# playHing/Scaled-MMD-GAN

Measured on AMD Instinct MI355X. Metric: images/sec/step (64x64 SMMD, batch 64) + MMD-kernel GB/s at 1/2/4/8 GPU, higher is better.
Workload: dtype fp32; 1 GPU; imagenet_smmd 64x64 SNResNet G/D, rbf kernel, scaling, SN, batch 64/GPU, 5D+1G schedule; model=snresnet, global_batch=64, parallelism=dp1, dp_mode=global, dp_forced=False, memory_format=nchw, miopen_winograd=True, miopen_find=False, step_graphs=False, conv_mean_pool=folded 4x4 stride-2 conv, miopen_db=/tmp/code/home/pair/home_parent/tmp/smmd_miopen_db_0gvd9db2

## Files before the change

### include/smmd_hip.h

```cpp
#ifndef SMMD_HIP_H
#define SMMD_HIP_H

#include <stddef.h>
#include <stdint.h>

#ifdef __cplusplus
extern "C" {
#endif

typedef enum {
    SMMD_OK = 0,
    SMMD_EINVAL = 1,
    SMMD_EHIP = 2,
    SMMD_EWORKSPACE = 3,
    SMMD_EUNSUPPORTED = 4
} smmd_status;

typedef void *smmd_stream_t;

typedef enum {
    SMMD_KIND_RBF = 0,
    SMMD_KIND_RQ = 1,
    SMMD_KIND_DISTANCE = 2,
    SMMD_KIND_DOT = 3
// ... 245 lines not shown
smmd_status smmd_cond_bn_relu_fwd(const float *x, const int32_t *labels, int N, int C, int HW,
                                  int num_classes, const float *scale, const float *offset,
                                  float eps, float *y, float *save, void *ws, size_t ws_bytes,
                                  smmd_stream_t stream);

smmd_status smmd_cond_bn_relu_bwd(const float *x, const float *gy, const int32_t *labels, int N,
                                  int C, int HW, int num_classes, const float *scale,
                                  const float *offset, const float *save, float *gx, float *gscale,
                                  float *goffset, void *ws, size_t ws_bytes, smmd_stream_t stream);

smmd_status smmd_conv3x3_thin(const float *x, const float *w, const float *bias, float *y,
                              int n, int ci, int co, int h, int w_img, int mode,
                              smmd_stream_t stream);

size_t smmd_conv3x3_thin_wgrad_workspace_bytes(int n, int ci, int co, int h, int w_img);

smmd_status smmd_conv3x3_thin_wgrad(const float *gy, const float *x, float *gw, int n, int ci,
                                    int co, int h, int w_img, void *ws, size_t ws_bytes,
                                    smmd_stream_t stream);

smmd_status smmd_conv3x3_thin_wgrad_acc(const float *gy, const float *x, float *gw, int n,
                                        int ci, int co, int h, int w_img, void *ws,
                                        size_t ws_bytes, smmd_stream_t stream);

int smmd_wino3x3_supported(int n, int ci, int ko, int h, int w_img);

size_t smmd_wino3x3_filter_bytes(int ko, int ci);

smmd_status smmd_wino3x3_filter(const float *w, int ko, int ci, int mode, float *u,
                                size_t u_bytes, smmd_stream_t stream);

size_t smmd_wino3x3_workspace_bytes(int n, int ci, int ko, int h, int w_img);

smmd_status smmd_wino3x3_conv(const float *x, const float *u, const float *bias, float *y, int n,
                              int ci, int ko, int h, int w_img, void *ws, size_t ws_bytes,
                              smmd_stream_t stream);

smmd_status smmd_wino3x3_conv_relu(const float *x, const float *u, const float *bias, float *y,
                                   int n, int ci, int ko, int h, int w_img, void *ws,
                                   size_t ws_bytes, smmd_stream_t stream);

smmd_status smmd_wino3x3_conv_mask(const float *x, const float *u, const float *bias,
                                   const float *mask, float *y, int n, int ci, int ko, int h,
                                   int w_img, void *ws, size_t ws_bytes, smmd_stream_t stream);

size_t smmd_wino3x3_conv2_workspace_bytes(int n, int ci, int ko, int h, int w_img);

smmd_status smmd_wino3x3_conv2(const float *x, const float *u, const float *x2, const float *u2,
                               const float *bias, float *y, int n, int ci, int ko, int h,
                               int w_img, void *ws, size_t ws_bytes, smmd_stream_t stream);

int smmd_wino4x4s2_supported(int n, int ci, int ko, int h, int w_img);

int smmd_wino4x4s2t_supported(int n, int k, int c, int hg, int wg);

size_t smmd_wino4x4s2_filter_bytes(int ko, int ci);

smmd_status smmd_wino4x4s2_filter(const float *w, int ko, int ci, float *u, size_t u_bytes,
                                  smmd_stream_t stream);

smmd_status smmd_wino4x4s2t_filter(const float *w, int k, int c, float *u, size_t u_bytes,
                                   smmd_stream_t stream);

size_t smmd_wino4x4s2_workspace_bytes(int n, int ci, int ko, int h, int w_img);

size_t smmd_wino4x4s2t_workspace_bytes(int n, int k, int c, int hg, int wg);

smmd_status smmd_wino4x4s2_conv(const float *x, const float *u, const float *bias, float *y,
                                int n, int ci, int ko, int h, int w_img, void *ws,
                                size_t ws_bytes, smmd_stream_t stream);

smmd_status smmd_wino4x4s2_conv_acc(const float *x, const float *u, const float *bias, float *y,
                                    int n, int ci, int ko, int h, int w_img, void *ws,
                                    size_t ws_bytes, smmd_stream_t stream);

smmd_status smmd_wino4x4s2t_conv(const float *gy, const float *u, const float *bias, float *dx,
                                 int n, int k, int c, int hg, int wg, void *ws, size_t ws_bytes,
                                 smmd_stream_t stream);

smmd_status smmd_wino4x4s2t_conv_mask(const float *gy, const float *u, const float *bias,
                                      const float *mask, float *dx, int n, int k, int c, int hg,
                                      int wg, void *ws, size_t ws_bytes, smmd_stream_t stream);

size_t smmd_wino4x4s2_conv2_workspace_bytes(int n, int ci, int ko, int h, int w_img);

smmd_status smmd_wino4x4s2_conv2(const float *x, const float *u, const float *x2,
                                 const float *u2, const float *bias, float *y, int n, int ci,
                                 int ko, int h, int w_img, void *ws, size_t ws_bytes,
                                 smmd_stream_t stream);

smmd_status smmd_wino3x3_filter_sn(const float *w, const float *sigma, const float *s, int ko,
                                   int ci, int mode, float *u, size_t u_bytes,
                                   smmd_stream_t stream);

smmd_status smmd_wino4x4s2_filter_sn(const float *w, const float *sigma, const float *s, int fold,
                                     int ko, int ci, float *u, size_t u_bytes,
                                     smmd_stream_t stream);

smmd_status smmd_wino4x4s2t_filter_sn(const float *w, const float *sigma, const float *s,
                                      int fold, int k, int c, float *u, size_t u_bytes,
                                      smmd_stream_t stream);

int smmd_wino3x3_wgrad_supported(int n, int ci, int co, int h, int w_img);


size_t smmd_wino3x3_wgrad_workspace_bytes(int n, int ci, int co, int h, int w_img);

smmd_status smmd_wino3x3_wgrad(const float *x, const float *gy, float *gw, int n, int ci, int co,
                               int h, int w_img, void *ws, size_t ws_bytes,
                               smmd_stream_t stream);

smmd_status smmd_wino3x3_wgrad_acc(const float *x, const float *gy, float *gw, int n, int ci,
                                   int co, int h, int w_img, void *ws, size_t ws_bytes,
                                   smmd_stream_t stream);

int smmd_wino4x4s2_wgrad_supported(int n, int ci, int co, int h, int w_img);

size_t smmd_wino4x4s2_wgrad_workspace_bytes(int n, int ci, int co, int h, int w_img);

smmd_status smmd_wino4x4s2_wgrad(const float *x, const float *gy, float *gw, int n, int ci,
                                 int co, int h, int w_img, void *ws, size_t ws_bytes,
                                 smmd_stream_t stream);

smmd_status smmd_wino4x4s2_wgrad_acc(const float *x, const float *gy, float *gw, int n, int ci,
                                     int co, int h, int w_img, void *ws, size_t ws_bytes,
                                     smmd_stream_t stream);

int smmd_conv1x1_supported(int n, int r, int m, int p);

size_t smmd_conv1x1_workspace_bytes(int n, int r, int m, int p);

smmd_status smmd_conv1x1(const float *a, const float *x, const float *bias, float *y, int n,
                         int r, int m, int p, void *ws, size_t ws_bytes, smmd_stream_t stream);

smmd_status smmd_conv1x1_t(const float *a, const float *x, const float *bias, float *y, int n,
                           int r, int m, int p, void *ws, size_t ws_bytes, smmd_stream_t stream);

int smmd_conv1x1_wgrad_supported(int n, int c, int k, int p);

size_t smmd_conv1x1_wgrad_workspace_bytes(int n, int c, int k, int p);

smmd_status smmd_conv1x1_wgrad(const float *gy, const float *x, float *gw, int n, int c, int k,
                               int p, void *ws, size_t ws_bytes, smmd_stream_t stream);

smmd_status smmd_conv1x1_wgrad_acc(const float *gy, const float *x, float *gw, int n, int c,
                                   int k, int p, void *ws, size_t ws_bytes,
                                   smmd_stream_t stream);

smmd_status smmd_gp_interp(const float *real, const float *fake, const float *alpha, float *out,
                           int b, int64_t per, int form, smmd_stream_t stream);

size_t smmd_gp_slope_workspace_bytes(int b, int c, int hw);

smmd_status smmd_gp_slope_fwd(const float *g, int b, int c, int hw, int channels_last, float eps,
                              float *out, float *slopes, void *ws, size_t ws_bytes,
                              smmd_stream_t stream);

smmd_status smmd_gp_slope_bwd(const float *g, const float *slopes, int b, int c, int hw,
                              int channels_last, const float *go, float *dg,
                              smmd_stream_t stream);

smmd_status smmd_critic_head_fwd(const float *d_real, int n_real, const float *d_fake, int n_fake,
                                 int kind, float *out, float *g_real, float *g_fake,
                                 float *gg_fake, smmd_stream_t stream);

size_t smmd_code_moments_workspace_bytes(int n, int dim);
// ... 10 lines not shown
```

### scaled-mmd-gan_amd/csrc/smmd_wino_s2.hip

```cpp
#include "smmd_wino_common.hpp"
#include "smmd_ldsdma.hpp"

namespace smmd {

namespace {

constexpr int S2_T = 256;
constexpr int S2_TB = 64;
constexpr int S2_KB = 64;
constexpr int S2_CC = 2;
constexpr int S2_STAGE = 9 * 8 * 64;
constexpr size_t S2_LDS = 2 * 2 * S2_STAGE * sizeof(float) + S2_KB * sizeof(float);

struct for_wino4x4s2_conv {};
struct for_wino4x4s2t_conv {};

__device__ __forceinline__ void s2_taps(const float *__restrict__ w, int64_t q, int fold,
                                        const float *__restrict__ sig,
                                        const float *__restrict__ sc, float (&f)[16]) {
#pragma clang fp contract(off)
    if (!sig) {
        const float *s = w + q * 16;
#pragma unroll
        for (int i = 0; i < 16; ++i) f[i] = s[i];
        return;
    }
    const float sigma = sig[0], scale = sc ? sc[0] : 1.f;
    if (!fold) {
        const float *s = w + q * 16;
#pragma unroll
        for (int i = 0; i < 16; ++i) f[i] = (s[i] / sigma) * scale;
        return;
    }
    const float *s = w + q * 9;
    float k[9];
#pragma unroll
    for (int j = 0; j < 9; ++j) k[j] = (s[j] / sigma) * scale;
#pragma unroll
    for (int si = 0; si < 4; ++si)
#pragma unroll
        for (int ti = 0; ti < 4; ++ti) {
            float acc = 0.f;
#pragma unroll
            for (int a = 0; a < 2; ++a)
#pragma unroll
                for (int b = 0; b < 2; ++b) {
                    const int uu = si - a, vv = ti - b;
                    if (uu >= 0 && uu < 3 && vv >= 0 && vv < 3) acc += k[uu * 3 + vv];
                }
            f[si * 4 + ti] = acc * 0.25f;
        }
}

__global__ void s2_filter_kernel(const float *__restrict__ w, int KO, int CI,
                                 float *__restrict__ u, const float *__restrict__ sig,
                                 const float *__restrict__ sc, int fold) {
    const int64_t idx = (int64_t)blockIdx.x * blockDim.x + threadIdx.x;
    if (idx >= (int64_t)KO * CI) return;
    const int ko = (int)(idx % KO), ci = (int)(idx / KO);
    float f[16];
    s2_taps(w, (int64_t)ko * CI + ci, fold, sig, sc, f);
    const int kb = ko >> 6, kl = ko & 63, cc = ci >> 1, h = ci & 1;
    const int64_t base = ((int64_t)kb * (CI >> 1) + cc) * 9;
    float r[9][4];
#pragma unroll
    for (int pi = 0; pi < 2; ++pi)
#pragma unroll
        for (int pj = 0; pj < 2; ++pj) {
            const float g00 = f[(pi) * 4 + pj], g01 = f[(pi) * 4 + 2 + pj];
            const float g10 = f[(2 + pi) * 4 + pj], g11 = f[(2 + pi) * 4 + 2 + pj];
            const float t[3][2] = {{g00, g01}, {g00 + g10, g01 + g11}, {g10, g11}};
#pragma unroll
            for (int i = 0; i < 3; ++i) {
                r[i * 3 + 0][2 * pi + pj] = t[i][0];
                r[i * 3 + 1][2 * pi + pj] = t[i][0] + t[i][1];
                r[i * 3 + 2][2 * pi + pj] = t[i][1];
            }
        }
    float4 *u4 = reinterpret_cast<float4 *>(u);
#pragma unroll
    for (int p = 0; p < 9; ++p)
        u4[((base + p) * 2 + h) * 64 + kl] = make_float4(r[p][0], r[p][1], r[p][2], r[p][3]);
// ... 508 lines not shown
    }

    const int64_t et = tile0 + th * 32 + l32;
    if (et >= g.T) return;
    const int en = (int)(et / g.Timg);
    const int er = (int)(et - (int64_t)en * g.Timg);
    const int ety = er / g.TW, etx = er - ety * g.TW;
    const int Hx = 2 * g.Hg, Wx = 2 * g.Wg;
    const int cl0 = kh * 32 + 4 * hl;
    const uint32_t o0 = (uint32_t)(((((int64_t)en * g.C + cb * 64 + cl0) * Hx + 4 * ety + qi) * Wx +
                                     4 * etx + qj) * 4);
    const uint32_t o1 = o0 + (uint32_t)Wx * 8;
    const uint32_t hw4 = (uint32_t)Hx * (uint32_t)Wx * 4;
    const __amdgpu_buffer_rsrc_t ds = buf_rsrc_2g(dx);
    float mk[16][4];
    const bool masked = g.mask != nullptr;
    if (masked) {
        const __amdgpu_buffer_rsrc_t ms = buf_rsrc_2g(g.mask);
#pragma unroll
        for (int r = 0; r < 16; r += 2) {
#pragma unroll
            for (int h = 0; h < 2; ++h) {
                const uint32_t so = (uint32_t)((r & 3) + 8 * (r >> 2) + h) * hw4;
                mk[r + h][0] = __builtin_bit_cast(float, __builtin_amdgcn_raw_buffer_load_b32(ms, o0, so, 0));
                mk[r + h][1] = __builtin_bit_cast(float, __builtin_amdgcn_raw_buffer_load_b32(ms, o0 + 8, so, 0));
                mk[r + h][2] = __builtin_bit_cast(float, __builtin_amdgcn_raw_buffer_load_b32(ms, o1, so, 0));
                mk[r + h][3] = __builtin_bit_cast(float, __builtin_amdgcn_raw_buffer_load_b32(ms, o1 + 8, so, 0));
            }
        }
    }
#ifdef S2_NO_EPI
    for (int r = 0; r < 2; r += 2) {
#else
#pragma unroll
    for (int r = 0; r < 16; r += 2) {
#endif
        const int cr = (r & 3) + 8 * (r >> 2);
#pragma unroll
        for (int h = 0; h < 2; ++h) {
            float m[9];
#pragma unroll
            for (int p = 0; p < 9; ++p) m[p] = acc[p][r + h];
            float s0[3], s1[3];
#pragma unroll
            for (int j = 0; j < 3; ++j) {
                s0[j] = m[j] + m[3 + j];
                s1[j] = m[3 + j] + m[6 + j];
            }
            const float b = Bs[cl0 + cr + h];
            float v[4] = {s0[0] + s0[1] + b, s0[1] + s0[2] + b, s1[0] + s1[1] + b,
                          s1[1] + s1[2] + b};
            if (masked) {
#pragma unroll
                for (int i = 0; i < 4; ++i) v[i] = mk[r + h][i] <= 0.f ? 0.f : v[i];
            }
            const uint32_t so = (uint32_t)(cr + h) * hw4;
            __builtin_amdgcn_raw_buffer_store_b32(__builtin_bit_cast(unsigned, v[0]), ds, o0, so, 0);
            __builtin_amdgcn_raw_buffer_store_b32(__builtin_bit_cast(unsigned, v[1]), ds, o0 + 8, so, 0);
            __builtin_amdgcn_raw_buffer_store_b32(__builtin_bit_cast(unsigned, v[2]), ds, o1, so, 0);
            __builtin_amdgcn_raw_buffer_store_b32(__builtin_bit_cast(unsigned, v[3]), ds, o1 + 8, so, 0);
        }
    }
}

template <bool EDGE>
__global__ __launch_bounds__(S2_T, 2) void s2t_conv_kernel(
    const float *__restrict__ gy, const float *__restrict__ u, const float *__restrict__ bias,
    float *__restrict__ dx, S2TGeom g) {
    uint32_t W = s2_xcd_order(blockIdx.x, gridDim.x);
    const int q = (int)(W & 3);
    W >>= 2;
    const int cb = (int)(W % (uint32_t)g.CB);
    W /= (uint32_t)g.CB;
    const int sl = (int)(W % (uint32_t)g.S);
    const int64_t tb = W / (uint32_t)g.S;
    switch (q) {
    case 0: s2t_body<EDGE, 0, 0>(gy, u, bias, dx, g, tb, cb, sl); break;
    case 1: s2t_body<EDGE, 0, 1>(gy, u, bias, dx, g, tb, cb, sl); break;
    case 2: s2t_body<EDGE, 1, 0>(gy, u, bias, dx, g, tb, cb, sl); break;
    default: s2t_body<EDGE, 1, 1>(gy, u, bias, dx, g, tb, cb, sl); break;
    }
}

}

static int s2_target() { return 256; }

static int s2t_slices(int64_t blocks, int nch) {
    int S = 1;
    while (blocks * S < s2_target() && nch / (2 * S) >= 4) S *= 2;
    return S;
}

static int s2_slices(int64_t blocks, int nch, int HWo) {
    int S = 1;
    while (blocks * S < s2_target() && nch / (2 * S) >= 8 && HWo % 4 == 0) S *= 2;
    return S;
}

}

using namespace smmd;

extern "C" int smmd_wino4x4s2_supported(int n, int ci, int ko, int h, int w_img) {
    return n > 0 && ci > 0 && ko > 0 && ci % S2_CC == 0 && ko % S2_KB == 0 && h > 0 &&
           w_img > 0 && h % 4 == 0 && w_img % 4 == 0 && (int64_t)n * ci * h * w_img < (1ll << 29) &&
           (int64_t)n * ko * h * w_img < (1ll << 31);
}

extern "C" size_t smmd_wino4x4s2_filter_bytes(int ko, int ci) {
    if (ko <= 0 || ci <= 0) return 0;
    return (size_t)36 * ko * ci * sizeof(float);
}

extern "C" smmd_status smmd_wino4x4s2_filter(const float *w, int ko, int ci, float *u,
                                             size_t u_bytes, smmd_stream_t stream) {
    if (ko <= 0 || ci <= 0 || !w || !u) return SMMD_EINVAL;
    if (ko % S2_KB || ci % S2_CC) return SMMD_EUNSUPPORTED;
    if (reinterpret_cast<uintptr_t>(u) & 15) return SMMD_EINVAL;
    if (u_bytes < smmd_wino4x4s2_filter_bytes(ko, ci)) return SMMD_EWORKSPACE;
    hipStream_t st = reinterpret_cast<hipStream_t>(stream);
    const int64_t n = (int64_t)ko * ci;
    s2_filter_kernel<<<dim3((unsigned)((n + 255) / 256)), dim3(256), 0, st>>>(w, ko, ci, u,
                                                                             nullptr, nullptr, 0);
    return last_launch_status();
}

extern "C" smmd_status smmd_wino4x4s2_filter_sn(const float *w, const float *sigma,
                                                const float *s, int fold, int ko, int ci,
                                                float *u, size_t u_bytes, smmd_stream_t stream) {
    if (ko <= 0 || ci <= 0 || !w || !u || !sigma || (fold != 0 && fold != 1)) return SMMD_EINVAL;
    if (ko % S2_KB || ci % S2_CC) return SMMD_EUNSUPPORTED;
    if (reinterpret_cast<uintptr_t>(u) & 15) return SMMD_EINVAL;
    if (u_bytes < smmd_wino4x4s2_filter_bytes(ko, ci)) return SMMD_EWORKSPACE;
    hipStream_t st = reinterpret_cast<hipStream_t>(stream);
    const int64_t n = (int64_t)ko * ci;
    s2_filter_kernel<<<dim3((unsigned)((n + 255) / 256)), dim3(256), 0, st>>>(w, ko, ci, u,
                                                                             sigma, s, fold);
    return last_launch_status();
}

extern "C" size_t smmd_wino4x4s2_workspace_bytes(int n, int ci, int ko, int h, int w_img) {
    if (!smmd_wino4x4s2_supported(n, ci, ko, h, w_img)) return 0;
    const int64_t T = (int64_t)n * (h / 4) * (w_img / 4);
    const int S = s2_slices(((T + S2_TB - 1) / S2_TB) * (ko / S2_KB), ci / S2_CC,
                            (h / 2) * (w_img / 2));
    return S > 1 ? (size_t)S * n * ko * (h / 2) * (w_img / 2) * sizeof(float) : 0;
}

static smmd_status s2_conv(const float *x, const float *u, const float *x2, const float *u2,
                           const float *bias, float *y, int n, int ci, int ko, int h, int w_img,
                           void *ws, size_t ws_bytes, smmd_stream_t stream, int acc = 0) {
    if (n < 0 || ci <= 0 || ko <= 0 || h < 0 || w_img < 0) return SMMD_EINVAL;
    if (n == 0 || h == 0 || w_img == 0) return SMMD_OK;
    if (!x || !u || !y || (!x2 != !u2)) return SMMD_EINVAL;
    if (!smmd_wino4x4s2_supported(n, ci, ko, h, w_img)) return SMMD_EUNSUPPORTED;
    if ((reinterpret_cast<uintptr_t>(x) | reinterpret_cast<uintptr_t>(y) |
         reinterpret_cast<uintptr_t>(u) | reinterpret_cast<uintptr_t>(x2) |
         reinterpret_cast<uintptr_t>(u2)) & 15)
        return SMMD_EINVAL;
    const int pair = x2 ? 2 : 1;
    S2Geom g{};
    g.x2 = x2;
    g.u2 = u2;
    g.N = n; g.C = ci; g.K = ko; g.H = h; g.W = w_img;
    g.TW = w_img / 4;
    g.Timg = (h / 4) * g.TW;
    g.T = (int64_t)n * g.Timg;
    const int64_t tb = (g.T + S2_TB - 1) / S2_TB;
    if (tb > 0x7fffffff) return SMMD_EINVAL;
    const int HWo = (h / 2) * (w_img / 2);
    const int S = s2_slices(tb * (ko / S2_KB), pair * ci / S2_CC, HWo);
    const int64_t total = (int64_t)n * ko * HWo;
    float *out = y;
// ... 43 lines not shown
extern "C" size_t smmd_wino4x4s2_conv2_workspace_bytes(int n, int ci, int ko, int h, int w_img) {
    if (!smmd_wino4x4s2_supported(n, ci, ko, h, w_img)) return 0;
    const int64_t T = (int64_t)n * (h / 4) * (w_img / 4);
    const int S = s2_slices(((T + S2_TB - 1) / S2_TB) * (ko / S2_KB), 2 * ci / S2_CC,
                            (h / 2) * (w_img / 2));
    return S > 1 ? (size_t)S * n * ko * (h / 2) * (w_img / 2) * sizeof(float) : 0;
}

extern "C" smmd_status smmd_wino4x4s2_conv2(const float *x, const float *u, const float *x2,
                                            const float *u2, const float *bias, float *y, int n,
                                            int ci, int ko, int h, int w_img, void *ws,
                                            size_t ws_bytes, smmd_stream_t stream) {
    if (!x2 || !u2) return SMMD_EINVAL;
    return s2_conv(x, u, x2, u2, bias, y, n, ci, ko, h, w_img, ws, ws_bytes, stream);
}

extern "C" int smmd_wino4x4s2t_supported(int n, int k, int c, int hg, int wg) {
    return n > 0 && k > 0 && c > 0 && k % 8 == 0 && c % 64 == 0 && hg > 0 && wg > 0 &&
           hg % 2 == 0 && wg % 2 == 0 && (int64_t)n * k * hg * wg < (1ll << 29) &&
           (int64_t)n * c * 4 * hg * wg < (1ll << 29);
}

extern "C" smmd_status smmd_wino4x4s2t_filter(const float *w, int k, int c, float *u,
                                              size_t u_bytes, smmd_stream_t stream) {
    if (k <= 0 || c <= 0 || !w || !u) return SMMD_EINVAL;
    if (k % 8 || c % 64) return SMMD_EUNSUPPORTED;
    if (reinterpret_cast<uintptr_t>(u) & 15) return SMMD_EINVAL;
    if (u_bytes < smmd_wino4x4s2_filter_bytes(k, c)) return SMMD_EWORKSPACE;
    hipStream_t st = reinterpret_cast<hipStream_t>(stream);
    const int64_t n = (int64_t)(k / 4) * c;
    s2t_filter_kernel<<<dim3((unsigned)((n + 255) / 256)), dim3(256), 0, st>>>(w, k, c, u,
                                                                              nullptr, nullptr, 0);
    return last_launch_status();
}

extern "C" smmd_status smmd_wino4x4s2t_filter_sn(const float *w, const float *sigma,
                                                 const float *s, int fold, int k, int c,
                                                 float *u, size_t u_bytes, smmd_stream_t stream) {
    if (k <= 0 || c <= 0 || !w || !u || !sigma || (fold != 0 && fold != 1)) return SMMD_EINVAL;
    if (k % 8 || c % 64) return SMMD_EUNSUPPORTED;
    if (reinterpret_cast<uintptr_t>(u) & 15) return SMMD_EINVAL;
    if (u_bytes < smmd_wino4x4s2_filter_bytes(k, c)) return SMMD_EWORKSPACE;
    hipStream_t st = reinterpret_cast<hipStream_t>(stream);
    const int64_t n = (int64_t)(k / 4) * c;
    s2t_filter_kernel<<<dim3((unsigned)((n + 255) / 256)), dim3(256), 0, st>>>(w, k, c, u,
                                                                              sigma, s, fold);
    return last_launch_status();
}

extern "C" size_t smmd_wino4x4s2t_workspace_bytes(int n, int k, int c, int hg, int wg) {
    if (!smmd_wino4x4s2t_supported(n, k, c, hg, wg)) return 0;
    const int64_t T = (int64_t)n * (hg / 2) * (wg / 2);
    const int S = s2t_slices(((T + S2_TB - 1) / S2_TB) * (c / 64) * 4, k / 8);
    return S > 1 ? (size_t)S * n * c * 4 * hg * wg * sizeof(float) : 0;
}

static smmd_status s2t_launch(const float *gy, const float *u, const float *bias,
                              const float *mask, float *dx, int n, int k, int c, int hg, int wg,
                              void *ws, size_t ws_bytes, smmd_stream_t stream) {
    if (n < 0 || k <= 0 || c <= 0 || hg < 0 || wg < 0) return SMMD_EINVAL;
    if (n == 0 || hg == 0 || wg == 0) return SMMD_OK;
    if (!gy || !u || !dx) return SMMD_EINVAL;
    if (!smmd_wino4x4s2t_supported(n, k, c, hg, wg)) return SMMD_EUNSUPPORTED;
    if ((reinterpret_cast<uintptr_t>(gy) | reinterpret_cast<uintptr_t>(dx) |
         reinterpret_cast<uintptr_t>(u) | reinterpret_cast<uintptr_t>(mask)) & 15)
        return SMMD_EINVAL;
    S2TGeom g{};
    g.N = n; g.K = k; g.C = c; g.Hg = hg; g.Wg = wg;
    g.TW = wg / 2;
    g.Timg = (hg / 2) * g.TW;
    g.T = (int64_t)n * g.Timg;
    const int64_t tb = (g.T + S2_TB - 1) / S2_TB;
    if (tb > 0x7fffffff) return SMMD_EINVAL;
    const int S = s2t_slices(tb * (c / 64) * 4, k / 8);
    const int64_t total = (int64_t)n * c * 4 * hg * wg;
    float *out = dx;
    if (S > 1) {
        if (!ws || ws_bytes < (size_t)S * total * sizeof(float)) return SMMD_EWORKSPACE;
        if (reinterpret_cast<uintptr_t>(ws) & 15) return SMMD_EINVAL;
        out = static_cast<float *>(ws);
    }
    static bool attr = false;
    if (!attr) {
        if (hipFuncSetAttribute(reinterpret_cast<const void *>(s2t_conv_kernel<false>),
                                hipFuncAttributeMaxDynamicSharedMemorySize,
                                (int)S2_LDS) != hipSuccess ||
            hipFuncSetAttribute(reinterpret_cast<const void *>(s2t_conv_kernel<true>),
                                hipFuncAttributeMaxDynamicSharedMemorySize,
                                (int)S2_LDS) != hipSuccess)
            return SMMD_EHIP;
        attr = true;
    }
    g.slab = S > 1 ? total : 0;
    g.CB = c / 64;
    g.S = S;
    g.mask = S > 1 ? nullptr : mask;

    hipStream_t st = reinterpret_cast<hipStream_t>(stream);
    const int64_t nblk = tb * (c / 64) * 4 * S;
    if (nblk > 0x7fffffff) return SMMD_EINVAL;
    const dim3 grid((unsigned)nblk);
    const float *b1 = S > 1 ? nullptr : bias;
    if (64 % g.TW == 0)
        s2t_conv_kernel<false><<<grid, dim3(S2_T), S2_LDS, st>>>(gy, u, b1, out, g);
    else
        s2t_conv_kernel<true><<<grid, dim3(S2_T), S2_LDS, st>>>(gy, u, b1, out, g);
    smmd_status e = last_launch_status();
    if (e != SMMD_OK || S == 1) return e;
    return slab_reduce_bias<for_wino4x4s2t_conv>(out, bias, dx, total / 4, S, c, 4 * hg * wg, 0,
                                                 mask, 0, st);
}

extern "C" smmd_status smmd_wino4x4s2t_conv(const float *gy, const float *u, const float *bias,
                                            float *dx, int n, int k, int c, int hg, int wg,
                                            void *ws, size_t ws_bytes, smmd_stream_t stream) {
    return s2t_launch(gy, u, bias, nullptr, dx, n, k, c, hg, wg, ws, ws_bytes, stream);
}

extern "C" smmd_status smmd_wino4x4s2t_conv_mask(const float *gy, const float *u,
                                                 const float *bias, const float *mask, float *dx,
                                                 int n, int k, int c, int hg, int wg, void *ws,
                                                 size_t ws_bytes, smmd_stream_t stream) {
    if (!mask) return SMMD_EINVAL;
    return s2t_launch(gy, u, bias, mask, dx, n, k, c, hg, wg, ws, ws_bytes, stream);
}
```

### scaled-mmd-gan_amd/gan/core/_lib.py

```python
from __future__ import annotations

import ctypes
import os
import threading

import torch

_PKG_ROOT = os.path.dirname(os.path.dirname(os.path.dirname(os.path.abspath(__file__))))
LIB_PATH = os.environ.get('SMMD_HIP_LIB', os.path.join(_PKG_ROOT, 'lib', 'libsmmd_hip.so'))
_CHECK_STAMP = 'SMMD_HIP_LIB' not in os.environ
CSRC = os.path.join(_PKG_ROOT, 'csrc')
HEADER = os.path.join(os.path.dirname(_PKG_ROOT), 'include', 'smmd_hip.h')

SMMD_MAX_TERMS = 8
SMMD_SN_MAX_LAYERS = 32
SN_P1_READY = 1
ADAM_SN_GDIRECT = 1
OPT_MAX_FUSED = 96
SN_MAX_FUSED = 16
ABI_VERSION = 17

KIND_RBF, KIND_RQ, KIND_DISTANCE, KIND_DOT = 0, 1, 2, 3
SMMD_EUNSUPPORTED = 4

# ... 69 lines not shown
    'smmd_smmd_loss_bwd': (_I, [_P, _I, _I, _I64, _P, _I, _P, _F, _I, _I, _P, _P, _P, _I, _P, _I,
                                _I, _P, _P, _P, _P, _P]),
    'smmd_scaled_loss_bwd': (_I, [_P, _I, _I, _I, _I64, _P, _I, _P, _F, _I, _I, _P, _P, _P, _P,
                                  _P]),
    'smmd_smmd_loss_fwd_gathered': (_I, [ctypes.POINTER(KernelDesc), _P, _I, _P, _I, _I, _I, _P,
                                         _I, _I, _F, _I, _I, _P, _P, _P, _P, _P, _P, _SZ, _P, _SZ,
                                         _P]),
    'smmd_smmd_loss_bwd_ex': (_I, [_P, _I, _I, _I, _I64, _P, _I, _P, _F, _I, _I, _P, _P, _P, _I,
                                   _P, _I, _I, _P, _P, _P, _P, _P]),
    'smmd_sn_workspace_bytes': (_SZ, [ctypes.POINTER(SnLayer), _I]),
    'smmd_sn_power_iter': (_I, [ctypes.POINTER(SnLayer), _I, _I, _F, _I, _P, _SZ, _P]),
    'smmd_sn_power_iter_ex': (_I, [ctypes.POINTER(SnLayer), _I, _I, _F, _I, _I, _P, _SZ, _P]),
    'smmd_sn_weight_bwd': (_I, [ctypes.POINTER(SnLayer), _I, _P, _SZ, _P]),
    'smmd_sn_grad_stats': (_I, [ctypes.POINTER(SnLayer), _I, _P, _SZ, _P]),
    'smmd_sn_clip_g': (_I, [ctypes.POINTER(SnLayer), _I, _F, _P, _SZ, _P]),
    'smmd_adam_flat_sn2': (_I, [_P, _P, _P, _P, ctypes.POINTER(ctypes.c_int64), _I, _F, _F, _F,
                                _F, _F, _F, _I64, _P, _P, _SZ, ctypes.POINTER(SnLayer),
                                ctypes.POINTER(ctypes.c_int32), _I, _P, _SZ, _I, _P]),
    'smmd_opt_workspace_bytes': (_SZ, [ctypes.POINTER(ctypes.c_int64), _I]),
    'smmd_clip_by_norm_flat': (_I, [_P, ctypes.POINTER(ctypes.c_int64), _I, _F, _P, _SZ, _P]),
    'smmd_adam_flat': (_I, [_P, _P, _P, _P, ctypes.POINTER(ctypes.c_int64), _I, _F, _F, _F, _F,
                            _F, _F, _I64, _P, _SZ, _P]),
    'smmd_adam_flat_sn': (_I, [_P, _P, _P, _P, ctypes.POINTER(ctypes.c_int64), _I, _F, _F, _F,
                               _F, _F, _F, _I64, _P, _SZ, ctypes.POINTER(SnLayer),
                               ctypes.POINTER(ctypes.c_int32), _I, _P, _SZ, _P]),
    'smmd_adam_flat_ex': (_I, [_P, _P, _P, _P, ctypes.POINTER(ctypes.c_int64), _I, _F, _F, _P,
                               _F, _F, _F, _P, _SZ, ctypes.POINTER(SnLayer),
                               ctypes.POINTER(ctypes.c_int32), _I, _P, _SZ, _P]),
    'smmd_poly_sums_workspace_bytes': (_SZ, [_I, _I, _I]),
    'smmd_poly_kernel_sums': (_I, [_P, _I, _P, _I, _I, ctypes.c_double, ctypes.c_double, _I, _P,
                                   _P, _P, _P, _P, _SZ, _P]),
    'smmd_poly_mmd2_var': (_I, [ctypes.POINTER(PolySums), ctypes.POINTER(PolySums),
                                ctypes.POINTER(PolySums), _I, ctypes.c_double, _I, _P, _P]),
    'smmd_fold_pool_weights': (_I, [ctypes.POINTER(_P), ctypes.POINTER(_P),
                                    ctypes.POINTER(ctypes.c_int64), _I, _I, _P]),
    'smmd_fold_up_weight': (_I, [_P, _P, _I, _I, _I, _P]),
    'smmd_conv1x1_supported': (_I, [_I, _I, _I, _I]),
    'smmd_conv1x1_workspace_bytes': (_SZ, [_I, _I, _I, _I]),
    'smmd_conv1x1': (_I, [_P, _P, _P, _P, _I, _I, _I, _I, _P, _SZ, _P]),
    'smmd_conv1x1_t': (_I, [_P, _P, _P, _P, _I, _I, _I, _I, _P, _SZ, _P]),
    'smmd_conv1x1_wgrad_supported': (_I, [_I, _I, _I, _I]),
    'smmd_conv1x1_wgrad_workspace_bytes': (_SZ, [_I, _I, _I, _I]),
    'smmd_conv1x1_wgrad': (_I, [_P, _P, _P, _I, _I, _I, _I, _P, _SZ, _P]),
    'smmd_conv1x1_wgrad_acc': (_I, [_P, _P, _P, _I, _I, _I, _I, _P, _SZ, _P]),
    'smmd_channel_sum_workspace_bytes': (_SZ, [_I, _I]),
    'smmd_channel_sum': (_I, [_P, _I, _I, _I, _P, _P, _SZ, _P]),
    'smmd_conv3x3_thin': (_I, [_P, _P, _P, _P, _I, _I, _I, _I, _I, _I, _P]),
    'smmd_mask_pool2': (_I, [_P, _P, _P, _P, _I, _P, _F, _F, _I64, _I, _I, _P, _P, _P]),
    'smmd_mask_pool2_adj': (_I, [_P, _P, _P, _F, _F, _I64, _I, _I, _P, _P]),
    'smmd_up_add': (_I, [_P, _P, _P, _P, _I, _I64, _I, _I, _P, _P]),
    'smmd_bn_relu_workspace_bytes': (_SZ, [_I, _I]),
    'smmd_bn_relu_fwd': (_I, [_P, _I, _I, _I, _P, _P, _P, _P, _F, _F, _P, _P, _SZ, _P]),
    'smmd_bn_relu_fwd_save': (_I, [_P, _I, _I, _I, _P, _P, _P, _P, _F, _F, _P, _P, _P, _SZ, _P]),
    'smmd_bn_relu_bwd': (_I, [_P, _P, _I, _I, _I, _P, _P, _P, _P, _P, _P, _SZ, _P]),
    'smmd_cond_bn_relu_workspace_bytes': (_SZ, [_I, _I]),
    'smmd_cond_bn_relu_fwd': (_I, [_P, _P, _I, _I, _I, _I, _P, _P, _F, _P, _P, _P, _SZ, _P]),
    'smmd_cond_bn_relu_bwd': (_I, [_P, _P, _P, _I, _I, _I, _I, _P, _P, _P, _P, _P, _P, _P, _SZ,
                                   _P]),
    'smmd_conv3x3_thin_wgrad_workspace_bytes': (_SZ, [_I, _I, _I, _I, _I]),
    'smmd_conv3x3_thin_wgrad': (_I, [_P, _P, _P, _I, _I, _I, _I, _I, _P, _SZ, _P]),
    'smmd_conv3x3_thin_wgrad_acc': (_I, [_P, _P, _P, _I, _I, _I, _I, _I, _P, _SZ, _P]),
    'smmd_wino3x3_supported': (_I, [_I, _I, _I, _I, _I]),
    'smmd_wino3x3_filter_bytes': (_SZ, [_I, _I]),
    'smmd_wino3x3_filter': (_I, [_P, _I, _I, _I, _P, _SZ, _P]),
    'smmd_wino3x3_workspace_bytes': (_SZ, [_I, _I, _I, _I, _I]),
    'smmd_wino3x3_conv': (_I, [_P, _P, _P, _P, _I, _I, _I, _I, _I, _P, _SZ, _P]),
    'smmd_wino3x3_conv_relu': (_I, [_P, _P, _P, _P, _I, _I, _I, _I, _I, _P, _SZ, _P]),
    'smmd_wino3x3_conv_mask': (_I, [_P, _P, _P, _P, _P, _I, _I, _I, _I, _I, _P, _SZ, _P]),
    'smmd_wino3x3_conv2_workspace_bytes': (_SZ, [_I, _I, _I, _I, _I]),
    'smmd_wino3x3_conv2': (_I, [_P, _P, _P, _P, _P, _P, _I, _I, _I, _I, _I, _P, _SZ, _P]),
    'smmd_wino4x4s2_supported': (_I, [_I, _I, _I, _I, _I]),
    'smmd_wino4x4s2t_supported': (_I, [_I, _I, _I, _I, _I]),
    'smmd_wino4x4s2_filter_bytes': (_SZ, [_I, _I]),
    'smmd_wino4x4s2_filter': (_I, [_P, _I, _I, _P, _SZ, _P]),
    'smmd_wino4x4s2t_filter': (_I, [_P, _I, _I, _P, _SZ, _P]),
    'smmd_wino4x4s2_workspace_bytes': (_SZ, [_I, _I, _I, _I, _I]),
    'smmd_wino4x4s2t_workspace_bytes': (_SZ, [_I, _I, _I, _I, _I]),
    'smmd_wino4x4s2_conv': (_I, [_P, _P, _P, _P, _I, _I, _I, _I, _I, _P, _SZ, _P]),
    'smmd_wino4x4s2_conv_acc': (_I, [_P, _P, _P, _P, _I, _I, _I, _I, _I, _P, _SZ, _P]),
    'smmd_wino4x4s2_conv2_workspace_bytes': (_SZ, [_I, _I, _I, _I, _I]),
    'smmd_wino4x4s2_conv2': (_I, [_P, _P, _P, _P, _P, _P, _I, _I, _I, _I, _I, _P, _SZ, _P]),
    'smmd_wino4x4s2t_conv': (_I, [_P, _P, _P, _P, _I, _I, _I, _I, _I, _P, _SZ, _P]),
    'smmd_wino4x4s2t_conv_mask': (_I, [_P, _P, _P, _P, _P, _I, _I, _I, _I, _I, _P, _SZ, _P]),
    'smmd_row_lrelu_sum': (_I, [_P, _P, _P, _P, _P, _I64, _I, _F, _P]),
    'smmd_row_lrelu_bcast': (_I, [_P, _P, _P, _P, _I64, _I, _F, _P]),
    'smmd_wino3x3_wgrad_supported': (_I, [_I, _I, _I, _I, _I]),
    'smmd_wino3x3_wgrad_workspace_bytes': (_SZ, [_I, _I, _I, _I, _I]),
    'smmd_wino3x3_wgrad': (_I, [_P, _P, _P, _I, _I, _I, _I, _I, _P, _SZ, _P]),
    'smmd_wino3x3_wgrad_acc': (_I, [_P, _P, _P, _I, _I, _I, _I, _I, _P, _SZ, _P]),
    'smmd_wino3x3_filter_sn': (_I, [_P, _P, _P, _I, _I, _I, _P, _SZ, _P]),
    'smmd_wino4x4s2_filter_sn': (_I, [_P, _P, _P, _I, _I, _I, _P, _SZ, _P]),
    'smmd_wino4x4s2t_filter_sn': (_I, [_P, _P, _P, _I, _I, _I, _P, _SZ, _P]),
    'smmd_wino4x4s2_wgrad_supported': (_I, [_I, _I, _I, _I, _I]),
    'smmd_wino4x4s2_wgrad_workspace_bytes': (_SZ, [_I, _I, _I, _I, _I]),
    'smmd_wino4x4s2_wgrad': (_I, [_P, _P, _P, _I, _I, _I, _I, _I, _P, _SZ, _P]),
    'smmd_wino4x4s2_wgrad_acc': (_I, [_P, _P, _P, _I, _I, _I, _I, _I, _P, _SZ, _P]),
    'smmd_poly_diff_ratio': (_I, [ctypes.POINTER(PolySums), ctypes.POINTER(PolySums),
                                  ctypes.POINTER(PolySums), ctypes.POINTER(PolySums), _I, _P,
                                  _P]),
    'smmd_gp_interp': (_I, [_P, _P, _P, _P, _I, _I64, _I, _P]),
    'smmd_gp_slope_workspace_bytes': (_SZ, [_I, _I, _I]),
    'smmd_gp_slope_fwd': (_I, [_P, _I, _I, _I, _I, _F, _P, _P, _P, _SZ, _P]),
    'smmd_gp_slope_bwd': (_I, [_P, _P, _I, _I, _I, _I, _P, _P, _P]),
    'smmd_critic_head_fwd': (_I, [_P, _I, _P, _I, _I, _P, _P, _P, _P, _P]),
    'smmd_code_moments_workspace_bytes': (_SZ, [_I, _I]),
    'smmd_code_moments': (_I, [_P, _I, _I, _P, _I, _P, _P, _P, _SZ, _P]),
}

EXPORTED_SYMBOLS = tuple(_SIGS)

_lock = threading.Lock()
_lib = None


def source_hash():
    import hashlib
    names = sorted(f for f in os.listdir(CSRC) if f.endswith(('.hip', '.hpp')))
    h = hashlib.sha256()
    for path in [os.path.join(CSRC, f) for f in names] + [HEADER]:
        with open(path, 'rb') as f:
            h.update(f.read())
    return h.hexdigest()[:16]


def lib():
    global _lib
    if _lib is not None:
        return _lib
    with _lock:
        if _lib is None:
            if not os.path.exists(LIB_PATH):
                raise SmmdLibraryError(
                    'libsmmd_hip.so not found at %s -- build it with '
                    '`python -c "import __graft_entry__ as g; g.build()"` or '
                    '`make -C scaled-mmd-gan_amd/csrc`' % LIB_PATH)
            try:
                handle = ctypes.CDLL(LIB_PATH, mode=ctypes.RTLD_GLOBAL)
            except OSError as e:
                raise SmmdLibraryError('failed to load %s: %s' % (LIB_PATH, e)) from e
            for name, (res, args) in _SIGS.items():
                fn = getattr(handle, name)
                fn.restype = res
                fn.argtypes = args
            if handle.smmd_abi_version() != ABI_VERSION:
                raise SmmdLibraryError('ABI version mismatch')
            if _CHECK_STAMP and os.path.isdir(CSRC):
                built, now = handle.smmd_source_hash().decode(), source_hash()
                if built != now:
                    raise SmmdLibraryError(
                        '%s was built from other sources (stamp %s, sources %s): rebuild '
                        'with `make -C scaled-mmd-gan_amd/csrc`' % (LIB_PATH, built, now))
            _lib = handle
    return _lib


def check(status: int, what: str):
    if status != 0:
        msg = lib().smmd_status_string(status).decode()
        raise SmmdError('%s failed: %s' % (what, msg))


def ptr(t):
    return None if t is None else ctypes.c_void_p(t.data_ptr())


def stream_handle(device=None):
# ... 113 lines not shown
```

Baseline: 6713 images/s.

## Add 8-wave stride-2 transposed Winograd conv kernel that splits MFMA phases across waves

```diff
diff --git a/include/smmd_hip.h b/include/smmd_hip.h
--- a/include/smmd_hip.h
+++ b/include/smmd_hip.h
@@ -351,6 +351,8 @@
                                       const float *mask, float *dx, int n, int k, int c, int hg,
                                       int wg, void *ws, size_t ws_bytes, smmd_stream_t stream);
 
+int smmd_wino4x4s2t_set_waves(int waves);
+
 size_t smmd_wino4x4s2_conv2_workspace_bytes(int n, int ci, int ko, int h, int w_img);
 
 smmd_status smmd_wino4x4s2_conv2(const float *x, const float *u, const float *x2,
diff --git a/scaled-mmd-gan_amd/csrc/smmd_wino_s2.hip b/scaled-mmd-gan_amd/csrc/smmd_wino_s2.hip
--- a/scaled-mmd-gan_amd/csrc/smmd_wino_s2.hip
+++ b/scaled-mmd-gan_amd/csrc/smmd_wino_s2.hip
@@ -1,3 +1,5 @@
+#include <stdlib.h>
+
 #include "smmd_wino_common.hpp"
 #include "smmd_ldsdma.hpp"
 
@@ -672,6 +674,294 @@
     }
 }
 
+constexpr int S2T8_T = 512;
+#ifndef S2T8_SLOT
+#define S2T8_SLOT 8
+#endif
+#ifndef S2T8_OCC
+#define S2T8_OCC 2
+#endif
+static_assert(4 * 9 * 2 * 64 * sizeof(float4) <= 2 * 2 * S2_STAGE * sizeof(float),
+              "the epilogue's accumulator exchange fits below the biases");
+
+template <bool EDGE, int QI, int QJ, int PH>
+__device__ __forceinline__ void s2t8_body(const float *__restrict__ gy, const float *__restrict__ u,
+                                          const float *__restrict__ bias, float *__restrict__ dx,
+                                          const S2TGeom &g, int64_t tb, int cb, int sl) {
+    extern __shared__ float4 s2_lds[];
+    float4 *const Vs = s2_lds;
+    float4 *const Us = s2_lds + 2 * (S2_STAGE / 4);
+    float *const Bs = reinterpret_cast<float *>(s2_lds + 4 * (S2_STAGE / 4));
+
+    const int tid = threadIdx.x, lane = tid & 63, w = tid >> 6;
+    constexpr int q = QI * 2 + QJ, qi = QI, qj = QJ;
+    constexpr int P0 = PH ? 5 : 0, NP = PH ? 4 : 5;
+    const int THg = g.Hg >> 1;
+    const int S = g.S;
+    const int64_t tile0 = tb * S2_TB;
+    const int nch = g.K / 8;
+    const int c0 = (int)((int64_t)nch * sl / S);
+    const int nchunk = (int)((int64_t)nch * (sl + 1) / S) - c0;
+    dx += (int64_t)sl * g.slab;
+
+    const int64_t gt = tile0 + lane;
+    const bool tok = gt < g.T;
+    int tn = 0, tty = 0, ttx = 0;
+    if (tok) {
+        tn = (int)(gt / g.Timg);
+        const int r = (int)(gt - (int64_t)tn * g.Timg);
+        tty = r / g.TW;
+        ttx = r - tty * g.TW;
+    }
+    const int64_t HW = (int64_t)g.Hg * g.Wg;
+    const float *gn = gy + ((int64_t)tn * g.K + (int64_t)c0 * 8 + w) * HW;
+    const float4 *ub = reinterpret_cast<const float4 *>(u) + (int64_t)q * g.C * g.K * 9 / 4 +
+                       ((int64_t)cb * nch + c0) * (S2_STAGE / 4);
+
+    f2v raw[3];
+    uint32_t roff[3];
+#pragma unroll
+    for (int a = 0; a < 3; ++a) {
+        const int yy = 2 * tty - 1 + qi + a;
+        roff[a] = (yy < 0 || yy >= g.Hg)
+                      ? BUF_OOB
+                      : (uint32_t)((((int64_t)tn * g.K + w) * HW + (int64_t)yy * g.Wg + 2 * ttx) * 4);
+    }
+    auto load_rows = [&](int cc) {
+        const __amdgpu_buffer_rsrc_t rs = buf_rsrc_2g(gy + ((int64_t)c0 + cc) * 8 * HW);
+#pragma unroll
+        for (int a = 0; a < 3; ++a)
+            raw[a] = __builtin_bit_cast(f2v, __builtin_amdgcn_raw_buffer_load_b64(rs, roff[a], 0, 0));
+    };
+    const int wu = __builtin_amdgcn_readfirstlane(w);
+    const uint32_t us_lds = lds_addr(Us);
+    auto load_u = [&](int cc) {
+        const float4 *sb = ub + (int64_t)cc * (S2_STAGE / 4);
+        const uint32_t dst = us_lds + (uint32_t)(cc & 1) * (S2_STAGE * 4);
+#pragma unroll
+        for (int i = 0; i < 3; ++i) {
+            const int piece = wu + 8 * i;
+            if (piece < S2_STAGE / 256)
+                glds16((uint32_t)(piece * 64 + lane) * 16, sb, dst + (uint32_t)piece * 1024);
+        }
+    };
+    f2v t[3];
+    float dd[3][3];
+    const bool eL = ttx == 0, eR = ttx == g.TW - 1;
+    auto xf_cols = [&](int cc) {
+        if constexpr (!EDGE) {
+            (void)cc;
+            t[0] = raw[0] - raw[1];
+            t[1] = raw[1];
+            t[2] = raw[2] - raw[1];
+        } else {
+            const float *gc = gn + (int64_t)cc * 8 * HW;
+#pragma unroll
+            for (int a = 0; a < 3; ++a) {
+                const int yy = 2 * tty - 1 + qi + a;
+                const bool row = (a == 0 && qi == 0) ? tty > 0
+                                 : (a == 2 && qi == 1) ? tty < THg - 1 : true;
+                const float cx = raw[a].x, cy = raw[a].y;
+                float L = dpp_from_left(cy), R = dpp_from_right(cx);
+                if (ttx > 0 && lane == 0) L = row ? gc[(int64_t)yy * g.Wg + 2 * ttx - 1] : 0.f;
+                if (ttx < g.TW - 1 && lane == 63)
+                    R = row ? gc[(int64_t)yy * g.Wg + 2 * ttx + 2] : 0.f;
+                L = ttx == 0 ? 0.f : L;
+                R = ttx == g.TW - 1 ? 0.f : R;
+                dd[a][0] = qj ? cx : L;
+                dd[a][1] = qj ? cy : cx;
+                dd[a][2] = qj ? R : cy;
+            }
+#pragma unroll
+            for (int b = 0; b < 3; ++b) {
+                const float t0 = dd[0][b] - dd[1][b], t2 = dd[2][b] - dd[1][b];
+                dd[0][b] = t0;
+                dd[2][b] = t2;
+            }
+        }
+    };
+    auto xf_row = [&](int i, int buf) {
+        float v[3];
+        if constexpr (!EDGE) {
+            if (qj == 0) {
+                const float ys = eR ? 0.f : t[i].y;
+                v[0] = dpp_from_left(ys) - t[i].x;
+                v[1] = t[i].x;
+                v[2] = t[i].y - t[i].x;
+            } else {
+                const float xs = eL ? 0.f : t[i].x;
+                v[0] = t[i].x - t[i].y;
+                v[1] = t[i].y;
+                v[2] = dpp_from_right(xs) - t[i].y;
+            }
+        } else {
+            v[0] = dd[i][0] - dd[i][1];
+            v[1] = dd[i][1];
+            v[2] = dd[i][2] - dd[i][1];
+        }
+        float *const Vl = reinterpret_cast<float *>(Vs + buf * (S2_STAGE / 4)) +
+                          ((w >> 2) * 64 + lane) * 4 + (w & 3);
+#pragma unroll
+        for (int j = 0; j < 3; ++j) Vl[(3 * i + j) * 512] = v[j];
+    };
+
+    f32x16 acc[NP];
+#pragma unroll
+    for (int p = 0; p < NP; ++p) acc[p] = f32x16{};
+
+    const int qd = w & 3, th = qd & 1, kh = qd >> 1, hl = lane >> 5, l32 = lane & 31;
+    const int ua = hl * 64 + kh * 32 + l32, vb = hl * 64 + th * 32 + l32;
+
+    const float bias_c = (bias && tid < 64) ? bias[cb * 64 + tid] : 0.f;
+    load_u(0);
+    load_rows(0);
+    xf_cols(0);
+#pragma unroll
+    for (int i = 0; i < 3; ++i) xf_row(i, 0);
+    if (tid < 64) Bs[tid] = bias_c;
+    dma_wait_all();
+    __syncthreads();
+    for (int cc = 0;; ++cc) {
+        const bool more = cc + 1 < nchunk;
+        const int buf = cc & 1, nbuf = buf ^ 1;
+        const float4 *U = Us + buf * (S2_STAGE / 4);
+        const float4 *V = Vs + buf * (S2_STAGE / 4);
+        float4 a = U[(P0 * 2) * 64 + ua], b = V[(P0 * 2) * 64 + vb];
+        __builtin_amdgcn_sched_barrier(0);
+        if (more) {
+            load_u(cc + 1);
+            __builtin_amdgcn_sched_barrier(0);
+            load_rows(cc + 1);
+            __builtin_amdgcn_sched_barrier(0);
+        }
+#pragma unroll
+        for (int p = 0; p < NP; ++p) {
+            const float4 ca = a, cb4 = b;
+#pragma unroll
+            for (int m = 0; m < 4; ++m) {
+                acc[p] = __builtin_amdgcn_mfma_f32_32x32x2f32(ca[m], cb4[m], acc[p], 0, 0, 0);
+                if (m == 0 && p < NP - 1) {
+                    a = U[((P0 + p + 1) * 2) * 64 + ua];
+                    b = V[((P0 + p + 1) * 2) * 64 + vb];
+                }
+                const int K = p * 4 + m;
+                if (more) {
+                    if (K == S2T8_SLOT) {
+                        asm volatile("" : "+v"(raw[0]), "+v"(raw[1]), "+v"(raw[2]));
+                        xf_cols(cc + 1);
+                    } else if (K == S2T8_SLOT + 2 || K == S2T8_SLOT + 4 || K == S2T8_SLOT + 6) {
+                        xf_row((K - S2T8_SLOT - 2) >> 1, nbuf);
+                    }
+                }
+                __builtin_amdgcn_sched_barrier(0);
+            }
+        }
+        if (!more) break;
+        dma_wait_all();
+        __syncthreads();
+    }
+
+    const int64_t et = tile0 + th * 32 + l32;
+    const bool eok = et < g.T;
+    const int en = eok ? (int)(et / g.Timg) : 0;
+    const int er = eok ? (int)(et - (int64_t)en * g.Timg) : 0;
+    const int ety = er / g.TW, etx = er - ety * g.TW;
+    const int Hx = 2 * g.Hg, Wx = 2 * g.Wg;
+    const int cl0 = kh * 32 + 4 * hl;
+    const uint32_t o0 = (uint32_t)(((((int64_t)en * g.C + cb * 64 + cl0) * Hx + 4 * ety + qi) * Wx +
+                                     4 * etx + qj) * 4);
+    const uint32_t o1 = o0 + (uint32_t)Wx * 8;
+    const uint32_t hw4 = (uint32_t)Hx * (uint32_t)Wx * 4;
+    const __amdgpu_buffer_rsrc_t ds = buf_rsrc_2g(dx);
+    float mk[8][4];
+    const bool masked = g.mask != nullptr;
+    if (masked) {
+        const __amdgpu_buffer_rsrc_t ms = buf_rsrc_2g(g.mask);
+        const uint32_t m0 = eok ? o0 : BUF_OOB, m1 = eok ? o1 : BUF_OOB;
+#pragma unroll
+        for (int rl = 0; rl < 8; ++rl) {
+            const int r = 8 * PH + rl;
+            const uint32_t so = (uint32_t)((r & 3) + 8 * (r >> 2)) * hw4;
+            mk[rl][0] = __builtin_bit_cast(float, __builtin_amdgcn_raw_buffer_load_b32(ms, m0, so, 0));
+            mk[rl][1] = __builtin_bit_cast(float, __builtin_amdgcn_raw_buffer_load_b32(ms, m0 + 8, so, 0));
+            mk[rl][2] = __builtin_bit_cast(float, __builtin_amdgcn_raw_buffer_load_b32(ms, m1, so, 0));
+            mk[rl][3] = __builtin_bit_cast(float, __builtin_amdgcn_raw_buffer_load_b32(ms, m1 + 8, so, 0));
+        }
+    }
+    __syncthreads();
+    float4 *const X = s2_lds;
+    constexpr int RO = 8 * (1 - PH);
+    constexpr int OP0 = PH ? 0 : 5, ONP = 9 - NP;
+#pragma unroll
+    for (int p = 0; p < NP; ++p)
+#pragma unroll
+        for (int r4 = 0; r4 < 2; ++r4)
+            X[((qd * 9 + P0 + p) * 2 + r4) * 64 + lane] =
+                make_float4(acc[p][RO + 4 * r4], acc[p][RO + 4 * r4 + 1], acc[p][RO + 4 * r4 + 2],
+                            acc[p][RO + 4 * r4 + 3]);
+    __syncthreads();
+#pragma unroll
+    for (int r4 = 0; r4 < 2; ++r4) {
+        float4 o4[ONP];
+#pragma unroll
+        for (int p = 0; p < ONP; ++p) o4[p] = X[((qd * 9 + OP0 + p) * 2 + r4) * 64 + lane];
+#pragma unroll
+        for (int rr = 0; rr < 4; ++rr) {
+            const int rl = 4 * r4 + rr, r = 8 * PH + rl;
+            const int cr = (r & 3) + 8 * (r >> 2);
+            float m[9];
+#pragma unroll
+            for (int p = 0; p < NP; ++p) m[P0 + p] = acc[p][r];
+#pragma unroll
+            for (int p = 0; p < ONP; ++p) m[OP0 + p] = o4[p][rr];
+            float s0[3], s1[3];
+#pragma unroll
+            for (int j = 0; j < 3; ++j) {
+                s0[j] = m[j] + m[3 + j];
+                s1[j] = m[3 + j] + m[6 + j];
+            }
+            const float b = Bs[cl0 + cr];
+            float v[4] = {s0[0] + s0[1] + b, s0[1] + s0[2] + b, s1[0] + s1[1] + b,
+                          s1[1] + s1[2] + b};
+            if (masked) {
+#pragma unroll
+                for (int i = 0; i < 4; ++i) v[i] = mk[rl][i] <= 0.f ? 0.f : v[i];
+            }
+            if (eok) {
+                const uint32_t so = (uint32_t)cr * hw4;
+                __builtin_amdgcn_raw_buffer_store_b32(__builtin_bit_cast(unsigned, v[0]), ds, o0, so, 0);
+                __builtin_amdgcn_raw_buffer_store_b32(__builtin_bit_cast(unsigned, v[1]), ds, o0 + 8, so, 0);
+                __builtin_amdgcn_raw_buffer_store_b32(__builtin_bit_cast(unsigned, v[2]), ds, o1, so, 0);
+                __builtin_amdgcn_raw_buffer_store_b32(__builtin_bit_cast(unsigned, v[3]), ds, o1 + 8, so, 0);
+            }
+        }
+    }
+}
+
+template <bool EDGE>
+__global__ __launch_bounds__(S2T8_T, S2T8_OCC) void s2t_conv8_kernel(
+    const float *__restrict__ gy, const float *__restrict__ u, const float *__restrict__ bias,
+    float *__restrict__ dx, S2TGeom g) {
+    uint32_t W = s2_xcd_order(blockIdx.x, gridDim.x);
+    const int q = (int)(W & 3);
+    W >>= 2;
+    const int cb = (int)(W % (uint32_t)g.CB);
+    W /= (uint32_t)g.CB;
+    const int sl = (int)(W % (uint32_t)g.S);
+    const int64_t tb = W / (uint32_t)g.S;
+    const int ph = __builtin_amdgcn_readfirstlane(threadIdx.x >> 8);
+    switch (q * 2 + ph) {
+    case 0: s2t8_body<EDGE, 0, 0, 0>(gy, u, bias, dx, g, tb, cb, sl); break;
+    case 1: s2t8_body<EDGE, 0, 0, 1>(gy, u, bias, dx, g, tb, cb, sl); break;
+    case 2: s2t8_body<EDGE, 0, 1, 0>(gy, u, bias, dx, g, tb, cb, sl); break;
+    case 3: s2t8_body<EDGE, 0, 1, 1>(gy, u, bias, dx, g, tb, cb, sl); break;
+    case 4: s2t8_body<EDGE, 1, 0, 0>(gy, u, bias, dx, g, tb, cb, sl); break;
+    case 5: s2t8_body<EDGE, 1, 0, 1>(gy, u, bias, dx, g, tb, cb, sl); break;
+    case 6: s2t8_body<EDGE, 1, 1, 0>(gy, u, bias, dx, g, tb, cb, sl); break;
+    default: s2t8_body<EDGE, 1, 1, 1>(gy, u, bias, dx, g, tb, cb, sl); break;
+    }
+}
+
 }
 
 static int s2_target() { return 256; }
@@ -680,6 +970,20 @@
     int S = 1;
     while (blocks * S < s2_target() && nch / (2 * S) >= 4) S *= 2;
     return S;
+}
+
+static int s2t_waves_now = -1;
+static int s2t_waves_setting() {
+    if (s2t_waves_now < 0) {
+        const char *e = getenv("SMMD_S2T_WAVES");
+        const int v = e ? atoi(e) : 0;
+        s2t_waves_now = (v == 4 || v == 8) ? v : 0;
+    }
+    return s2t_waves_now;
+}
+static int s2t_waves(int64_t blocks) {
+    const int v = s2t_waves_setting();
+    return v ? v : blocks <= s2_target() ? 8 : 4;
 }
 
 static int s2_slices(int64_t blocks, int nch, int HWo) {
@@ -889,13 +1193,14 @@
     }
     static bool attr = false;
     if (!attr) {
-        if (hipFuncSetAttribute(reinterpret_cast<const void *>(s2t_conv_kernel<false>),
-                                hipFuncAttributeMaxDynamicSharedMemorySize,
-                                (int)S2_LDS) != hipSuccess ||
-            hipFuncSetAttribute(reinterpret_cast<const void *>(s2t_conv_kernel<true>),
-                                hipFuncAttributeMaxDynamicSharedMemorySize,
-                                (int)S2_LDS) != hipSuccess)
-            return SMMD_EHIP;
+        const void *ks[4] = {reinterpret_cast<const void *>(s2t_conv_kernel<false>),
+                             reinterpret_cast<const void *>(s2t_conv_kernel<true>),
+                             reinterpret_cast<const void *>(s2t_conv8_kernel<false>),
+                             reinterpret_cast<const void *>(s2t_conv8_kernel<true>)};
+        for (const void *k : ks)
+            if (hipFuncSetAttribute(k, hipFuncAttributeMaxDynamicSharedMemorySize, (int)S2_LDS) !=
+                hipSuccess)
+                return SMMD_EHIP;
         attr = true;
     }
     g.slab = S > 1 ? total : 0;
@@ -908,14 +1213,23 @@
     if (nblk > 0x7fffffff) return SMMD_EINVAL;
     const dim3 grid((unsigned)nblk);
     const float *b1 = S > 1 ? nullptr : bias;
-    if (64 % g.TW == 0)
-        s2t_conv_kernel<false><<<grid, dim3(S2_T), S2_LDS, st>>>(gy, u, b1, out, g);
-    else
-        s2t_conv_kernel<true><<<grid, dim3(S2_T), S2_LDS, st>>>(gy, u, b1, out, g);
+    const bool edge = 64 % g.TW != 0;
+    if (s2t_waves(nblk) == 8) {
+        auto k8 = edge ? s2t_conv8_kernel<true> : s2t_conv8_kernel<false>;
+        k8<<<grid, dim3(S2T8_T), S2_LDS, st>>>(gy, u, b1, out, g);
+    } else {
+        auto k4 = edge ? s2t_conv_kernel<true> : s2t_conv_kernel<false>;
+        k4<<<grid, dim3(S2_T), S2_LDS, st>>>(gy, u, b1, out, g);
+    }
     smmd_status e = last_launch_status();
     if (e != SMMD_OK || S == 1) return e;
     return slab_reduce_bias<for_wino4x4s2t_conv>(out, bias, dx, total / 4, S, c, 4 * hg * wg, 0,
                                                  mask, 0, st);
+}
+
+extern "C" int smmd_wino4x4s2t_set_waves(int waves) {
+    s2t_waves_now = (waves == 4 || waves == 8) ? waves : -1;
+    return s2t_waves_setting();
 }
 
 extern "C" smmd_status smmd_wino4x4s2t_conv(const float *gy, const float *u, const float *bias,
diff --git a/scaled-mmd-gan_amd/gan/core/_lib.py b/scaled-mmd-gan_amd/gan/core/_lib.py
--- a/scaled-mmd-gan_amd/gan/core/_lib.py
+++ b/scaled-mmd-gan_amd/gan/core/_lib.py
@@ -175,6 +175,7 @@
     'smmd_wino4x4s2_conv2': (_I, [_P, _P, _P, _P, _P, _P, _I, _I, _I, _I, _I, _P, _SZ, _P]),
     'smmd_wino4x4s2t_conv': (_I, [_P, _P, _P, _P, _I, _I, _I, _I, _I, _P, _SZ, _P]),
     'smmd_wino4x4s2t_conv_mask': (_I, [_P, _P, _P, _P, _P, _I, _I, _I, _I, _I, _P, _SZ, _P]),
+    'smmd_wino4x4s2t_set_waves': (_I, [_I]),
     'smmd_row_lrelu_sum': (_I, [_P, _P, _P, _P, _P, _I64, _I, _F, _P]),
     'smmd_row_lrelu_bcast': (_I, [_P, _P, _P, _P, _I64, _I, _F, _P]),
     'smmd_wino3x3_wgrad_supported': (_I, [_I, _I, _I, _I, _I]),
```

After: 6750 images/s, median of 4. About the same (+0.6%).
